# YamaneKoyo/mri-to-speech

Hardware: AMD Instinct MI355X
Metric: rtMRI frames/s end-to-end (256x256 frames -> 64-bin mel -> 11413 Hz wav) (higher is better)
Workload: dtype bf16x3; 1 GPU; e2e rtMRI->wav, 64 clips x 30 frames per GPU at 256x256 (configs[3] per-GPU share); clips_per_gpu=64, frames_per_clip=30, global_batch_clips=64, hw=256, parallelism=dp1, chunk=1920

## Files before the change

### mri-to-speech_amd/csrc/conv_gemm.hip

```cpp
#include "conv_igemm.hpp"

#include <cstring>
#include <map>
#include <mutex>

#include "prof.hpp"

namespace m2s {
namespace {

__device__ __attribute__((aligned(16))) uint4 g_zero_page[4];

template <int N>
__device__ __forceinline__ void wait_vm() {
  asm volatile("s_waitcnt vmcnt(%0)" ::"n"(N) : "memory");
}

__device__ __forceinline__ void dma16(const void* src, void* lds_wave_base) {
  __builtin_amdgcn_global_load_lds(src, lds_wave_base, 16, 0, 0);
}

__device__ __forceinline__ bf16x8 lrelu_frag(bf16x8 v, float slope) {
  uint4 u = __builtin_bit_cast(uint4, v);
  uint32_t w[4] = {u.x, u.y, u.z, u.w};
// ... 82 lines not shown
}

__device__ __forceinline__ void ld4f(const bf16_t* p, float* v) {
  const uint2 u = *reinterpret_cast<const uint2*>(p);
  v[0] = __uint_as_float(u.x << 16);
  v[1] = __uint_as_float(u.x & 0xffff0000u);
  v[2] = __uint_as_float(u.y << 16);
  v[3] = __uint_as_float(u.y & 0xffff0000u);
}

constexpr int ROW = 64;

__device__ __forceinline__ int swz_f(int x) { return (0x1320 >> (4 * x)) & 3; }
__device__ __forceinline__ int swz(int row, int chunk) { return row * ROW + ((chunk ^ swz_f((row >> 2) & 3)) << 4); }

template <int BM, int BN, int MT, int NT, int S, int KIND, int XF, int SP>
__global__ void __launch_bounds__(256, (BN >= 256 || (BM >= 256 && BN >= 128) ? 2 : 1)) conv_gemm_kernel(const ConvBatch ab, int n_tiles, int se_imgs,
                                                                                                      float* __restrict__ kpart) {
  const ConvArgs a = ab.a[KIND == KIND_CONV1D ? blockIdx.z : 0];
  constexpr int WN = BN / (NT * 16);
  constexpr int WM = 4 / WN;
  static_assert(WM * WN == 4 && WM * MT * 16 == BM, "bad tile");
  constexpr int R = SP == 1 ? 2 : 1;
  constexpr int A_PER_WAVE = BM / 64;
  constexpr int B_BLOCKS = BN / 16;
  constexpr int B_PER_WAVE = (B_BLOCKS + 3) / 4;
  constexpr int SLOT = (R * (BM + BN) + 16) * ROW;
  constexpr int PER_STAGE = R * (A_PER_WAVE + B_PER_WAVE);
  constexpr bool PRE = SP == 1 && XF == IN_SE_SCALE;
  constexpr bool SE = XF == IN_SE_SCALE;
  extern __shared__ __attribute__((aligned(16))) char smem[];
// ... 320 lines not shown
  }
  }

  if (nks > 1) {
    float* __restrict__ P = kpart + ((size_t)blockIdx.z * nks + ks) * a.M * a.cs_out;
#pragma unroll
    for (int mi = 0; mi < MT; ++mi) {
      const int m = m0 + wm * MT * 16 + mi * 16 + r16;
      if (m >= a.M) continue;
#pragma unroll
      for (int ni = 0; ni < NT; ++ni) {
        const int n4 = n0 + wn * NT * 16 + ni * 16 + 4 * g;
        if (n4 < a.cs_out)
          *reinterpret_cast<float4*>(P + (size_t)m * a.cs_out + n4) =
              make_float4(acc[ni][mi][0], acc[ni][mi][1], acc[ni][mi][2], acc[ni][mi][3]);
      }
    }
    return;
  }

  bf16_t* __restrict__ Y = static_cast<bf16_t*>(a.y);
  const bf16_t* __restrict__ Rs = static_cast<const bf16_t*>(a.res);
#pragma unroll
  for (int mi = 0; mi < MT; ++mi) {
    const int m = m0 + wm * MT * 16 + mi * 16 + r16;
    if (m >= a.M) continue;
    long orow;
    if constexpr (KIND == KIND_CONVT) {
      const int b = m / a.L_in, qq = m - (m / a.L_in) * a.L_in;
      orow = (long)b * a.L_out + (long)qq * a.ct_u + phase;
// ... 207 lines not shown
  }
  return static_cast<float*>(b.first);
}

const char* kname(int k) {
  switch (k) {
    case KIND_CONV2D: return "conv2d";
    case KIND_CONV1D: return "conv1d";
    case KIND_CONVT: return "convT";
    default: return "gemm";
  }
}

inline int se_images(int BM, int OH) { return BM % OH == 0 ? BM / OH : OH % BM == 0 ? 1 : (BM + OH - 1) / OH + 1; }

template <int BM, int BN, int MT, int NT, int KIND, int XF, int SP, int SF = 0>
void launch_tile(const ConvBatch& b, hipStream_t s, int phases, double flops, double bytes) {
  const ConvArgs& a = b.a[0];
  constexpr int S = SF ? SF : SP == 1 ? (BM == 128 && BN == 64 && XF != IN_SE_SCALE ? 3 : 2) : (BN >= 256 || BM + BN >= 384) ? 2 : (BM >= 256 ? 3 : 4);
  constexpr int R = SP == 1 ? 2 : 1;
  allow_lds(reinterpret_cast<const void*>(&conv_gemm_kernel<BM, BN, MT, NT, S, KIND, XF, SP>));
  const int m_tiles = ceil_div(a.M, BM), n_tiles = ceil_div(a.cs_out, BN);
  int se_imgs = 0;
  if (a.in_xform == IN_SE_SCALE) {
    M2S_CHECK(KIND == KIND_GEMM && a.OH > 0 && a.cs_in % 8 == 0, "SE scale needs the GEMM kind with OH = rows per image");
    se_imgs = se_images(BM, a.OH);
  }
  const size_t lds = (size_t)S * (R * (BM + BN) + 16) * ROW + (size_t)se_imgs * a.cs_in * sizeof(float);
  M2S_CHECK(lds <= 160 * 1024, "conv_gemm: LDS budget");
  int nst = 0;
  for (int i = 0; i < (KIND == KIND_CONV1D ? phases : 1); ++i) nst = std::max(nst, b.a[i].kp / 32);
  const int tiles = m_tiles * n_tiles * phases;
  const int slots = device_cus() * std::max(1, std::min(2, (int)(160 * 1024 / lds)));
  const char* fe = getenv("M2S_KSPLIT");
  const int force = fe ? atoi(fe) : 0;
  int nks = 1;
  if (force > 0)
    nks = std::min(force, std::max(1, nst));
  else if (2 * tiles <= slots && nst >= 8) {
    const char* mx = getenv("M2S_KSPLIT_MAX");
    const char* ms = getenv("M2S_KSPLIT_MINST");
    nks = std::max(1, std::min({slots / tiles, nst / (ms ? std::max(1, atoi(ms)) : 4), mx ? std::max(1, atoi(mx)) : 8}));
  }
  const size_t part_bytes = (size_t)phases * nks * a.M * a.cs_out * sizeof(float);
  if (nks > 1 && part_bytes > ((size_t)256 << 20)) nks = 1;
  float* kpart = nks > 1 ? ksplit_scratch(s, part_bytes) : nullptr;
  if (!kpart) nks = 1;
  dim3 grid(m_tiles * n_tiles, nks, phases);
  char name[96];
  static const bool detail = getenv("M2S_PROF_DETAIL") != nullptr;
  if (detail)
    snprintf(name, sizeof(name), "conv_gemm<%s,%dx%d%s> K%d N%d M%d", kname(KIND), BM, BN, SP == 1 ? ",x3" : SP == 2 ? ",e4m3" : "", a.kp, a.cs_out, a.M);
  else
    snprintf(name, sizeof(name), "conv_gemm_kernel<%d, %d, %d, %d, %d, %d, %d, %d>", BM, BN, MT, NT, S, KIND, XF, SP);
  {
    ProfScope ps(name, flops, bytes, s);
    hipLaunchKernelGGL((conv_gemm_kernel<BM, BN, MT, NT, S, KIND, XF, SP>), grid, dim3(256), lds, s, b, n_tiles, se_imgs, kpart);
  }
// ... 79 lines not shown
    const ConvArgs& c = as[i];
    M2S_CHECK(c.kind == a.kind && c.M == a.M && c.cs_in == a.cs_in && c.cs_out == a.cs_out && c.n_pad == a.n_pad &&
                  c.in_xform == a.in_xform && c.L_in == a.L_in && c.L_out == a.L_out,
              "conv_gemm batch: convs of one shape");
    M2S_CHECK(c.kp % 32 == 0 && c.kp >= c.ntaps * c.cs_in && c.ntaps <= 31, "conv_gemm batch: kp / taps");
    M2S_CHECK(c.x && c.w && c.bias && c.y && c.y != c.x && c.y != c.res, "conv_gemm batch: operand pointers");
    for (int j = 0; j < i; ++j) M2S_CHECK(as[j].y != c.y, "conv_gemm batch: two convs write one output");
    M2S_CHECK((double)(c.M / c.L_out) * c.L_in * c.cs_in * 2 < 2147483647.0, "conv_gemm batch: 32-bit offsets");
    b.a[i] = c;
  }
  if (a.M <= 0) return;
  launch_kind<KIND_CONV1D, 1>(a, s, n, flops, bytes, &b);
  M2S_HIP(hipGetLastError());
}

void launch_conv_gemm(const ConvArgs& a, bool split, hipStream_t s, double flops, double bytes) {
  M2S_CHECK(a.cs_in % 8 == 0 && a.cs_out % 4 == 0, "conv_gemm: channel strides");
  M2S_CHECK(a.cs_in >= 32 ? a.cs_in % 32 == 0 : 32 % a.cs_in == 0, "conv_gemm: channel stride vs the 32-wide K step");
  M2S_CHECK(a.ntaps <= 31, "conv_gemm: at most 31 taps");
  {
    const double in_elems = a.kind == KIND_CONV2D ? (double)(a.M / (a.OH * a.OW)) * a.IH * a.IW * a.cs_in
                            : a.kind == KIND_CONV1D ? (double)(a.M / a.L_out) * a.L_in * a.cs_in
                            : a.kind == KIND_CONVT  ? (double)a.M * a.cs_in
                                                    : (double)a.M * a.cs_in;
    M2S_CHECK(in_elems * (split ? 2 : 1) < 2147483647.0, "conv_gemm: input too large for 32-bit offsets (use a smaller chunk)");
  }
  M2S_CHECK(a.kp % 32 == 0 && a.kp >= a.ntaps * a.cs_in, "conv_gemm: kp");
  M2S_CHECK(a.kind != KIND_CONV2D || a.ks == 3, "conv_gemm: 2-D kernels are 3x3 (1x1 runs as GEMM)");
  if (a.M <= 0) return;
  M2S_CHECK(!(split && a.wscale), "conv_gemm: e4m3 operands take bf16 storage");
// ... 35 lines not shown
```

### mri-to-speech_amd/csrc/conv_igemm.hpp

```cpp
#pragma once

#include "m2s_common.hpp"

namespace m2s {

enum ConvKind { KIND_CONV2D = 0, KIND_CONV1D = 1, KIND_CONVT = 2, KIND_GEMM = 3 };
enum Act { ACT_NONE = 0, ACT_SILU = 1, ACT_LRELU = 2, ACT_SIGMOID = 3 };
enum InXform { IN_NONE = 0, IN_LRELU = 1, IN_SE_SCALE = 2 };

struct ConvArgs {
  const void* x;
  const void* w;
  const float* bias;
  const void* res;
  void* y;
  const void* in_scale;
  const float* wscale;
  int kind;
  int M;
  int cs_in, cs_out;
  int n_pad;
  int kp;
  int ntaps;
  int tpc;
// ... 5 lines not shown
  int accum;
  float accum_div;
  float res_unslope;
  int act_after_res;
  int kwave;
};

constexpr int CONV_BATCH = 3;
struct ConvBatch {
  ConvArgs a[CONV_BATCH];
};

template <typename T>
void launch_conv(const ConvArgs& a, hipStream_t s, double flops = 0.0, double bytes = 0.0);
void launch_conv_gemm(const ConvArgs& a, bool split, hipStream_t s, double flops, double bytes);
void launch_conv_gemm_batch(const ConvArgs* a, int n, hipStream_t s, double flops, double bytes);
bool conv_halo_supported(const ConvArgs& a);
void launch_conv_halo(const ConvArgs& a, hipStream_t s, double flops, double bytes);

inline int conv_tpc(int cs_in, int kc) { return cs_in < kc ? kc / cs_in : 1; }
inline int conv_kp(int ntaps, int cs_in, int kc) {
  int tpc = conv_tpc(cs_in, kc);
  return round_up(ntaps, tpc) * cs_in;
}

}
```

### mri-to-speech_amd/csrc/kernels.hpp

```cpp
#pragma once

#include "m2s_common.hpp"

namespace m2s {

enum AsyncCode : unsigned { M2S_ASYNC_LSTM = 1u, M2S_ASYNC_WS = 2u };
struct AsyncReport {
  unsigned spin_max = 1u << 20;
  unsigned* err = nullptr;
};
__device__ __forceinline__ void report_async(unsigned* err, unsigned code, int lane) {
  if (err && lane == 0) __hip_atomic_store(err, code, __ATOMIC_RELAXED, __HIP_MEMORY_SCOPE_SYSTEM);
}

template <typename T>
void launch_stem(const float* frames, int N, int H, int W, int OH, int OW, int pad_t, int pad_l,
                 const float* w9, const float* bias, int cout, int cs_out, T* y, hipStream_t s);

int dw_pixel_blocks(int OH, int OW);
template <typename T>
void launch_dwconv(const T* x, int N, int IH, int IW, int OH, int OW, int stride, int pad_t, int pad_l,
                   int C, int cs, const float* w9, const float* bias, T* y, float* sums, hipStream_t s);

template <typename T>
// ... 6 lines not shown
                    const void* w8 = nullptr, const float* wsc = nullptr, int kp8 = 0);
void launch_rows_e4m3(const void* x, long rows, int cs, void* y8, int ld8, hipStream_t s);

bool se_gemm_f8_supported(int P, int cs_in, int cs_out);
void launch_se_gemm_f8(const void* x8, int M, int P, int cs_in, const void* w8, int kp, int n_pad, const float* wscale,
                       const float* bias, const void* gate, const void* res, void* y, int cs_out, hipStream_t s,
                       double flops, double bytes, void* y8 = nullptr, int ld8 = 0);

bool se_gemm_sp_supported(int P, int cs_in, int cs_out);
void launch_se_gemm_sp(const void* x, int M, int P, int cs_in, const void* w, int n_pad, const float* bias,
                       const void* gate, const void* res, void* y, int cs_out, hipStream_t s, double flops, double bytes);

bool se_ws_supported(int P, int cs_in, int cs_out);
void launch_se_ws(const void* x, int M, int P, int cs_in, const void* w, int n_pad, const float* bias, const void* gate,
                  const void* res, void* y, int cs_out, hipStream_t s, double flops, double bytes, AsyncReport rep = {},
                  bool x_f32 = false);

bool se_ws_f8_supported(int P, int cs_in, int cs_out);
void launch_se_ws_f8(const void* x8, int M, int P, int cs_in, const void* w8, int kp, int n_pad, const float* wscale,
                     const float* bias, const void* gate, const void* res, void* y, int cs_out, hipStream_t s, double flops,
                     double bytes, void* y8 = nullptr, int ld8 = 0, AsyncReport rep = {});

bool ir_ws_supported(int H, int W, int cs_in, int kp, int cs_mid);
bool ir_ws_s2_supported(int H, int W, int cs_in, int kp, int cs_mid, int OH, int OW, int pad_t, int pad_l);
void launch_ir_ws(const void* x, int N, int H, int W, int cs_in, int kp, int cs_mid, const void* wpw, const float* bpw,
                  const float* wdw, const float* bdw, void* y, void* se_mean, double flops, double bytes,
                  hipStream_t s, AsyncReport rep = {}, int stride = 1, int OH = 0, int OW = 0, int pad_t = 0,
                  int pad_l = 0, double spill = 0.0, bool fm32 = false);
int ir_s2band_bands(int OH);
bool ir_s2band_supported(int IH, int IW, int OH, int OW, int cs_in, int kp, int cs_mid);
void launch_ir_s2band(const void* x, int N, int IH, int IW, int cs_in, int kp, const void* wpw, const float* bpw,
// ... 160 lines not shown
```

### mri-to-speech_amd/csrc/model.cpp

```cpp
#include "model.hpp"

#include <algorithm>
#include <cmath>
#include <cstdlib>
#include <cstring>
#include <initializer_list>
#include <type_traits>
#include <utility>

#include "pack.hpp"
#include "prof.hpp"

namespace m2s {

void Arena::upload(int device) {
  M2S_HIP(hipSetDevice(device));
  M2S_HIP(hipMalloc(&dev_, host_.size() + 256));
  M2S_HIP(hipMemcpy(dev_, host_.data(), host_.size(), hipMemcpyHostToDevice));
  std::vector<uint8_t>().swap(host_);
}

Arena::~Arena() {
  if (dev_) (void)hipFree(dev_);
}
// ... 2 lines not shown
  if (const char* e = std::getenv(name)) v = std::strcmp(e, "0") != 0;
}
static void env_int(const char* name, int& v) {
  if (const char* e = std::getenv(name)) v = std::atoi(e);
}

Acoustic::Acoustic(const StateDict& sd, int n_mels, int hidden, int dtype, int device)
    : dtype_(dtype), device_(device), n_mels_(n_mels), hidden_(hidden) {
  for (auto [name, v] : std::initializer_list<std::pair<const char*, bool*>>{
           {"M2S_IR_FUSED", &ir_fused_},   {"M2S_IR_WS", &ir_ws_},         {"M2S_IR_WS_S2", &ir_ws_s2_},
           {"M2S_IRWS_F32", &irws_f32_},   {"M2S_STEM_FUSED", &stem_fused_}, {"M2S_F8_EXPAND", &f8_expand_},
           {"M2S_F8_S2", &f8_s2_},         {"M2S_F8_ER", &f8_er_},         {"M2S_ER8_X8", &er8_x8_},
           {"M2S_F8_ER2", &f8_er2_},       {"M2S_SE_Y8", &se_y8_},         {"M2S_SE_FUSED", &se_fused_},
           {"M2S_ER_FUSED", &er_fused_},   {"M2S_SE_WS", &se_ws_},         {"M2S_LSTM_PERSISTENT", &lstm_persistent_},
           {"M2S_LSTM_MID", &lstm_mid_},   {"M2S_LSTM_X3", &lstm_x3_},     {"M2S_LSTM_X3G", &lstm_x3g_},
           {"M2S_SE_SP", &se_sp_},         {"M2S_ER_MRG", &er_mrg_},       {"M2S_IR_S2BAND", &ir_s2band_}})
    env_flag(name, *v);
  env_int("M2S_IRWS_MIN", irws_min_);
  env_int("M2S_SEWS_MIN", sews_min_cus_);
  pack_acoustic(sd, n_mels, hidden, dtype, arena_, p_);
  arena_.upload(device);
  for (auto& b : p_.blocks) {
    b.c1.resolve(arena_);
    if (b.type != 0) b.c2.resolve(arena_);
    if (b.type == 2) {
      b.se1.resolve(arena_);
      b.se2.resolve(arena_);
    }
  }
  p_.lstm_ih.resolve(arena_);
  M2S_HIP(hipHostMalloc(reinterpret_cast<void**>(&err_host_), sizeof(unsigned), hipHostMallocMapped | hipHostMallocCoherent));
// ... 161 lines not shown
  } else if (std::is_same<T, bf16_t>::value && er_fused_ && b.er_frag && b.stride == 2 &&
             ers2_fused_supported(nh, nw, b.c1.cs_in, b.mid, chan_stride(b.cout), b.c1.kp, b.c2.kp)) {
    uint8_t* y8 = er8_next && ((chan_stride(b.cout) == 32 && p_.blocks[k + 1].er8 && er8_fused_supported(nh, nw, 32, 128, 32)) ||
                               (chan_stride(b.cout) == 64 && p_.blocks[k + 1].er8w && er8w_fused_supported(nh, nw, 64, 224, b.cout)))
                      ? er8_next
                      : nullptr;
    launch_ers2_fused(reinterpret_cast<const bf16_t*>(cur), nc, oh, ow, nh, nw, qt, ql, b.c1.cs_in, b.mid,
                      chan_stride(b.cout), static_cast<const bf16_t*>(arena_.ptr(b.er_wexp)), b.c1.b,
                      static_cast<const bf16_t*>(arena_.ptr(b.er_wpwl)), b.c2.b, reinterpret_cast<bf16_t*>(nxt),
                      2.0 * px * b.mid * (9.0 * b.cin + b.cout),
                      2.0 * ((double)nc * oh * ow * b.c1.cs_in + px * chan_stride(b.cout)) + (y8 ? px * 32 : 0.0), s, y8);
    next8 = y8;
  } else {
    ConvArgs a = conv2d_args(p, b.c1, cur, M);
    a.act = ACT_SILU;
    run_conv<T>(a, b.c1, s);
    ConvArgs q = conv_args(b.c2);
    q.x = M;
    q.y = nxt;
    q.M = nc * nh * nw;
    q.OH = nh * nw;
    q.res = b.skip ? cur : nullptr;
    run_conv<T>(q, b.c2, s);
  }
}

template <typename T>
void Acoustic::effnet_ir_front(EffPass<T>& p, size_t k) {
  const Block& b = p_.blocks[k];
  const int nc = p.nc, oh = p.oh, ow = p.ow, nh = p.nh, nw = p.nw, qt = p.qt, ql = p.ql;
  T *const cur = p.cur, *const M = p.b.M, *const M2 = p.b.M2, *const se_mean = p.b.se_mean;
  float* const sums = p.b.sums;
  uint8_t *&cur8 = p.cur8, *const *const X8 = p.b.X8;
  hipStream_t s = p.s;
  const int cs = chan_stride(b.mid);
  constexpr bool SPL = std::is_same<T, sp_t>::value;
  const bool FUSABLE = (std::is_same<T, bf16_t>::value && (dtype_ == M2S_DT_BF16 || dtype_ == M2S_DT_FP8)) || SPL;
// ... 125 lines not shown
                        (next8 ? rows * b.cout : 0.0),
                    next8, ld8, ws_report());
  } else if (f8) {
    const double rows = (double)nc * nh * nw, co = chan_stride(b.cout);
    launch_se_gemm_f8(M2, nc * nh * nw, nh * nw, cs, arena_.ptr(b.f8_w), b.f8_kp, b.f8_npad,
                      static_cast<const float*>(arena_.ptr(b.f8_s)), static_cast<const float*>(arena_.ptr(b.f8_b)),
                      scale, b.skip ? cur : nullptr, nxt, chan_stride(b.cout), s, 2.0 * rows * b.mid * b.cout,
                      rows * cs + 2.0 * rows * co * (b.skip ? 2.0 : 1.0) + (double)b.f8_npad * b.f8_kp +
                          2.0 * nc * cs + (next8 ? rows * ld8 : 0.0),
                      next8, ld8);
  } else if (sews) {
    const double rows = (double)nc * nh * nw;
    launch_se_ws(M2, nc * nh * nw, nh * nw, cs, b.c2.w, b.c2.n_pad, b.c2.b, scale, b.skip ? cur : nullptr, nxt,
                 chan_stride(b.cout), s, 2.0 * rows * b.mid * b.cout,
                 4.0 * rows * b.mid + 4.0 * rows * b.cout * (b.skip ? 2.0 : 1.0) + 4.0 * b.cout * b.mid + 4.0 * nc * b.mid,
                 ws_report(), mid_f32);
  } else if (SPL && se_sp_ && se_gemm_sp_supported(nh * nw, cs, chan_stride(b.cout))) {
    const double rows = (double)nc * nh * nw, co = chan_stride(b.cout);
    launch_se_gemm_sp(M2, nc * nh * nw, nh * nw, cs, b.c2.w, b.c2.n_pad, b.c2.b, scale, b.skip ? cur : nullptr, nxt,
                      chan_stride(b.cout), s, 2.0 * rows * b.mid * b.cout,
                      4.0 * rows * cs + 4.0 * rows * co * (b.skip ? 2.0 : 1.0) + 4.0 * b.c2.n_pad * b.c2.kp +
                          4.0 * nc * cs);
  } else {
    ConvArgs q = conv_args(b.c2);
    q.x = M2;
    q.y = nxt;
    q.M = nc * nh * nw;
    q.OH = nh * nw;
    q.in_xform = IN_SE_SCALE;
    q.in_scale = scale;
    q.res = b.skip ? cur : nullptr;
// ... 979 lines not shown
```

### mri-to-speech_amd/csrc/model.hpp

```cpp
#pragma once

#include <map>
#include <string>
#include <vector>

#include "../../include/m2s.h"
#include "conv_igemm.hpp"
#include "kernels.hpp"

namespace m2s {

struct HostTensor {
  const float* data = nullptr;
  std::vector<int64_t> shape;
  size_t numel() const {
    size_t n = 1;
    for (auto d : shape) n *= (size_t)d;
    return n;
  }
};
using StateDict = std::map<std::string, HostTensor>;
StateDict make_state_dict(const m2s_tensor* t, int n);

class Arena {
// ... 196 lines not shown
  bool irws_f32_ = true;
  int sews_min_cus_ = 1;
  bool stem_fused_ = true;
  bool f8_er_ = true;
  bool se_y8_ = true;
  bool f8_er2_ = true;
  bool er8_x8_ = true;
  bool f8_expand_ = true;
  bool f8_s2_ = true;
  bool se_fused_ = true;
  bool er_fused_ = true;
  bool se_sp_ = false;
  bool se_ws_ = true;
  bool er_mrg_ = true;
  bool ir_s2band_ = true;
  bool lstm_persistent_ = true;
  bool lstm_mid_ = true;
  bool lstm_x3_ = true;
  bool lstm_x3g_ = true;

  size_t workspace_bytes(int B, int T, int H, int W) const;
  void forward(const float* frames, int B, int T, int H, int W, float* mel_norm, Workspace& ws, hipStream_t s);
  void effnet(const float* frames, int N, int H, int W, float* feats, int stop_after, float* probe, int* probe_dims,
              Workspace& ws, hipStream_t s);
  void bilstm(const float* feats, int B, int T, float* y, float* mel_norm, Workspace& ws, hipStream_t s);
  size_t ragged_workspace_bytes(const int* lengths, int B, int H, int W) const;
  void bilstm_ragged(const float* feats, const int* lengths, int B, long N, float* y, float* mel_norm, Workspace& ws,
                     hipStream_t s);
  void forward_ragged(const float* frames, const int* lengths, int B, long N, int H, int W, float* mel_norm,
                      Workspace& ws, hipStream_t s);
// ... 163 lines not shown
```

### mri-to-speech_amd/csrc/se_ws.hip

```cpp
#include <cstdlib>
#include <cstring>

#include "kernels.hpp"
#include "prof.hpp"

namespace m2s {
namespace {

typedef uint32_t u32x4 __attribute__((ext_vector_type(4)));

constexpr int ROWB = 128;

__device__ __attribute__((aligned(16))) uint4 g_se_ws_zero[4];


__device__ __forceinline__ void dma16(const void* src, uint32_t lds_wave_base) {
  unsigned keep;
  asm volatile("s_mov_b32 %0, m0\n\ts_mov_b32 m0, %2\n\ts_nop 0\n\tglobal_load_lds_dwordx4 %1, off\n\ts_mov_b32 m0, %0"
               : "=&s"(keep)
               : "v"(src), "s"(lds_wave_base)
               : "memory");
}
__device__ __forceinline__ uint32_t lds_u32(const void* p) { return (uint32_t)(uintptr_t)p; }

// ... 25 lines not shown
  unsigned spin_max;
  unsigned* err;
};

constexpr int E8M0_ONE = 0x7f7f7f7f;
typedef int i32x8 __attribute__((ext_vector_type(8)));
template <bool F8>
__device__ __forceinline__ int swz_k(int r) { return F8 ? (((r >> 1) & 1) | (r & 4)) : (r & 6); }
__device__ __forceinline__ int gate4_f8(int d, const float* s) {
  const f32x2_t lo = __builtin_amdgcn_cvt_pk_f32_fp8(d, false);
  const f32x2_t hi = __builtin_amdgcn_cvt_pk_f32_fp8(d, true);
  const int r = __builtin_amdgcn_cvt_pk_fp8_f32(lo[0] * s[0], lo[1] * s[1], 0, false);
  return __builtin_amdgcn_cvt_pk_fp8_f32(hi[0] * s[2], hi[1] * s[3], r, true);
}

template <int WM, int WN, int NT, int NL, int NS, int IF, bool F8, bool XF = false>
__global__ void __launch_bounds__(64 * (WM * WN + NL), 1) se_ws_kernel(const SeWsArgs a) {
  static_assert(!(F8 && XF), "fp32 activations: split engine");
  constexpr int NC = WM * WN;
  constexpr int BM = 64 * WM, BN = 16 * NT * WN, MT = 4;
  constexpr int BLK = (BN + BM) / 8;
  static_assert(BLK % NL == 0, "DMA blocks per loader");
  constexpr int PER = BLK / NL;
  static_assert((IF + 1) * PER <= 63 && IF >= 1 && IF <= NS - 1, "steps in flight per loader within vmcnt");
  constexpr int SLOT = (BN + BM) * ROWB;
  extern __shared__ __attribute__((aligned(16))) char smem[];

  const int tid = threadIdx.x, lane = tid & 63;
  const int wave = __builtin_amdgcn_readfirstlane(tid >> 6);
  const int nimg = BM / a.P > 0 ? BM / a.P : 1;
  const int grow = F8 ? a.cs_in * 2 : a.cs_in * 4;
  const int gimg = (grow + 1023) / 1024 * 1024;
  char* gbuf = smem + NS * SLOT;
  unsigned* flags = reinterpret_cast<unsigned*>(gbuf + 2 * nimg * gimg);
  const uint32_t full0 = lds_u32(flags), free0 = lds_u32(flags + NS), poison = lds_u32(flags + 2 * NS);
  const int nsteps = F8 ? a.kp / 128 : a.cs_in / 32;
  const int n_tiles = a.n_tiles_m;
  const int my_tiles = (int)blockIdx.x < n_tiles ? (n_tiles - 1 - (int)blockIdx.x) / (int)gridDim.x + 1 : 0;
  auto tile_rows = [&](int tile, int& m0, int& mend) {
    m0 = tile < a.full_tiles ? tile * BM : a.full_tiles * BM + (tile - a.full_tiles) * (BM / 2);
    mend = min(m0 + (tile < a.full_tiles ? BM : BM / 2), a.M);
  };

  if (tid <= 2 * NS) flags[tid] = 0u;
  __syncthreads();

  if (wave >= NC) {
    const int l = wave - NC;
    const char* zp = reinterpret_cast<const char*>(g_se_ws_zero);
    const int lrow = lane >> 3, pch = lane & 7;
    const int wrow_b = F8 ? a.kp : a.cs_in * 4, wlo = a.cs_in * 2, xrow_b = F8 ? a.cs_in : a.cs_in * 4;
    int s = 0;
    for (int it = 0; it < my_tiles; ++it) {
      const int tile = blockIdx.x + it * gridDim.x;
      int m0, mend;
      tile_rows(tile, m0, mend);
      const uint8_t* xt = a.x + (size_t)m0 * xrow_b;
      for (int st = 0; st < nsteps; ++st, ++s) {
        const int slot = s % NS, use = s / NS;
        if (use > 0 && !wait_flag(free0 + 4 * slot, (unsigned)(NC * use), a.spin_max)) {
          report_async(a.err, M2S_ASYNC_WS, lane);
          if (lane == 0) asm volatile("ds_write_b32 %0, %1\n\ts_waitcnt lgkmcnt(0)" ::"v"(poison), "v"(1u) : "memory");
        }
        if (st == 0 && l == 0) {
          const int img0 = m0 / a.P, nb = grow / 16;
          char* gdst = gbuf + (it & 1) * nimg * gimg;
          for (int im = 0; im < nimg; ++im)
            for (int o = 0; o < gimg / 16; o += 64) {
              const int e = o + lane;
// ... 39 lines not shown

  const int wm = wave / WN, wn = wave % WN;
  const int g = lane >> 4, r16 = lane & 15;
  const int sw = swz_k<F8>(r16);
  const uint32_t ch0 = (uint32_t)(((F8 ? 2 * g : g) ^ sw) << 4), ch1 = (uint32_t)(((F8 ? 2 * g + 1 : g + 4) ^ sw) << 4);
  const uint32_t sm0 = lds_u32(smem);
  const uint32_t a_lds0 = sm0 + (uint32_t)((wn * NT * 16 + r16) * ROWB);
  const uint32_t b_lds0 = sm0 + (uint32_t)((BN + wm * 64 + r16) * ROWB);
  const uint32_t bx0 = XF ? b_lds0 + (uint32_t)(((2 * g) ^ swz_k<true>(r16)) << 4) : 0u;
  const uint32_t bx1 = XF ? b_lds0 + (uint32_t)(((2 * g + 1) ^ swz_k<true>(r16)) << 4) : 0u;
  const uint32_t wa0 = XF ? a_lds0 + ch0 : 0u, wa1 = XF ? a_lds0 + ch1 : 0u;
  const uint32_t g_lds0 = lds_u32(gbuf) + (uint32_t)(g * (F8 ? 64 : 16));
  bool bad = false;
  int s = 0;
  for (int it = 0; it < my_tiles; ++it) {
    const int tile = blockIdx.x + it * gridDim.x;
    int m0, mend;
    tile_rows(tile, m0, mend);
    const bool active = m0 + wm * 64 < mend;
    const int wimg = (min(m0 + wm * 64, a.M - 1)) / a.P - m0 / a.P;
    const uint32_t gl = g_lds0 + (uint32_t)(((it & 1) * nimg + wimg) * gimg);
    f32x4 acc[NT][MT];
#pragma unroll
    for (int ni = 0; ni < NT; ++ni)
#pragma unroll
      for (int mi = 0; mi < MT; ++mi) acc[ni][mi] = f32x4{0.f, 0.f, 0.f, 0.f};

    for (int st = 0; st < nsteps; ++st, ++s) {
      const int slot = s % NS, use = s / NS;
      if (!wait_flag(full0 + 4 * slot, (unsigned)(NL * (use + 1)), a.spin_max)) {
        report_async(a.err, M2S_ASYNC_WS, lane);
// ... 210 lines not shown
        unpack_bf16x4(rv[mi & 1][ni][0], r);
        unpack_bf16x4(rv[mi & 1][ni][1], rl);
        float v[4] = {acc[ni][mi][0] + bb.x + (r[0] + rl[0]), acc[ni][mi][1] + bb.y + (r[1] + rl[1]),
                      acc[ni][mi][2] + bb.z + (r[2] + rl[2]), acc[ni][mi][3] + bb.w + (r[3] + rl[3])};
        if (bad) v[0] = v[1] = v[2] = v[3] = __builtin_nanf("");
        uint2 hi, lo;
        split4(v, hi, lo);
        bf16_t* yo = Y + (size_t)m * a.cs_out * 2 + n4;
        *reinterpret_cast<uint2*>(yo) = hi;
        *reinterpret_cast<uint2*>(yo + a.cs_out) = lo;
      }
    }
  }
}

template <int WM, int WN, int NT, int NL, int NS, int IF, bool F8 = false, bool XF = false>
void launch_cfg(SeWsArgs& a, hipStream_t s, double flops, double bytes) {
  static_assert(IF <= 3, "tail waits");
  constexpr int BM = 64 * WM, BN = 16 * NT * WN;
  const void* fn = reinterpret_cast<const void*>(&se_ws_kernel<WM, WN, NT, NL, NS, IF, F8, XF>);
  allow_lds(fn);
  const int nimg = BM / a.P > 0 ? BM / a.P : 1;
  const int gimg = ((F8 ? a.cs_in * 2 : a.cs_in * 4) + 1023) / 1024 * 1024;
  const size_t lds = (size_t)NS * (BN + BM) * ROWB + (size_t)2 * nimg * gimg + (2 * NS + 1) * sizeof(unsigned);
  M2S_CHECK(lds <= 160 * 1024, "se_ws: LDS budget");
  M2S_CHECK(BM % a.P == 0 || a.P % BM == 0, "se_ws: tile rows vs image size");
  M2S_CHECK(a.cs_out <= BN, "se_ws: one n tile covers the outputs");
  M2S_CHECK((F8 ? a.kp / 128 : a.cs_in / 32) >= NS, "se_ws: K steps per tile >= ring slots (gate rows are double-buffered per tile)");
  const int tiles = ceil_div(a.M, BM), G = std::min(tiles, device_cus());
  const int full = tiles / G * G, rem = tiles - full;
  const bool halve = rem > 0 && 2 * rem <= G && (BM / 2) % 64 == 0 && ((BM / 2) % a.P == 0 || a.P % (BM / 2) == 0) &&
                     getenv("M2S_SEWS_HALF") && atoi(getenv("M2S_SEWS_HALF")) == 1;
  a.full_tiles = halve ? full : tiles;
  a.n_tiles_m = halve ? full + 2 * rem : tiles;
  const dim3 grid(G);
  char name[72];
  if (XF)
    snprintf(name, sizeof(name), "se_ws_kernel<%d, %d, %d, %d, %d, %d, false, true>", WM, WN, NT, NL, NS, IF);
  else
    snprintf(name, sizeof(name), "se_ws_kernel<%d, %d, %d, %d, %d, %d, %s>", WM, WN, NT, NL, NS, IF,
             F8 ? "true" : "false");
  ProfScope ps(name, flops, bytes, s);
  hipLaunchKernelGGL((se_ws_kernel<WM, WN, NT, NL, NS, IF, F8, XF>), grid, dim3(64 * (WM * WN + NL)), lds, s, a);
  M2S_HIP(hipGetLastError());
}

}

bool se_ws_supported(int P, int cs_in, int cs_out) {
  return cs_in % 32 == 0 && cs_in / 32 >= 5 && ((P % 256 == 0 && cs_out <= 128) || (P == 64 && cs_out > 128 && cs_out <= 224));
}

void launch_se_ws(const void* x, int M, int P, int cs_in, const void* w, int n_pad, const float* bias, const void* gate,
                  const void* res, void* y, int cs_out, hipStream_t s, double flops, double bytes, AsyncReport rep,
                  bool x_f32) {
  M2S_CHECK(se_ws_supported(P, cs_in, cs_out) && M % P == 0 && cs_out % 4 == 0, "se_ws: unsupported shape");
  M2S_CHECK(x && w && bias && gate && y && y != res && y != x, "se_ws: operand pointers");
  M2S_CHECK((double)M * cs_in * 4 < 2147483647.0 * 2, "se_ws: input too large");
  if (M <= 0) return;
  SeWsArgs a;
  std::memset(&a, 0, sizeof(a));
  a.x = static_cast<const uint8_t*>(x);
  a.w = static_cast<const uint8_t*>(w);
  a.bias = bias;
  a.gate = static_cast<const uint8_t*>(gate);
  a.res = static_cast<const bf16_t*>(res);
  a.y = static_cast<bf16_t*>(y);
  a.M = M;
  a.P = P;
  a.cs_in = cs_in;
  a.cs_out = cs_out;
  a.spin_max = rep.spin_max;
  a.err = rep.err;
  static const int cfg = [] {
    const char* e = std::getenv("M2S_SE_WS_CFG");
    return e ? std::atoi(e) : 0;
  }();
  if (x_f32) {
    if (cs_out <= 128) {
      M2S_CHECK(n_pad >= 128, "se_ws: weight rows");
      return launch_cfg<4, 1, 8, 4, 3, 2, false, true>(a, s, flops, bytes);
    }
    M2S_CHECK(n_pad >= 224, "se_ws: weight rows");
    return launch_cfg<2, 2, 7, 4, 3, 2, false, true>(a, s, flops, bytes);
  }
  if (cs_out <= 128) {
    M2S_CHECK(n_pad >= 128, "se_ws: weight rows");
    switch (cfg) {
      case 1: return launch_cfg<4, 2, 4, 2, 3, 1>(a, s, flops, bytes);
      case 2: return launch_cfg<2, 2, 4, 4, 4, 2>(a, s, flops, bytes);
      case 3: return launch_cfg<2, 2, 4, 4, 4, 1>(a, s, flops, bytes);
      case 4: return launch_cfg<4, 2, 4, 4, 3, 2>(a, s, flops, bytes);
      default: return launch_cfg<4, 1, 8, 4, 3, 2>(a, s, flops, bytes);
    }
  } else {
    M2S_CHECK(n_pad >= 224, "se_ws: weight rows");
    switch (cfg) {
      case 1: return launch_cfg<2, 2, 7, 2, 3, 1>(a, s, flops, bytes);
      default: return launch_cfg<2, 2, 7, 4, 3, 2>(a, s, flops, bytes);
// ... 46 lines not shown
```

Baseline: 51080 rtMRI frames/s.

## Fuse stride-2 expand conv with projection GEMM and reverse se_ws tile walk

Adds an epilogue variant to the split 128x128 conv2d kernel that applies bias and SiLU to the expand-conv tile, stages it in LDS as hi/lo bf16, and runs the 1x1 projection GEMM in the same block. Stride-2 inverted-residual blocks then use one launch and skip the global round trip of the mid activation. Separately, the se_ws persistent kernel gains a REV template flag that walks tiles in reverse order, presumably to improve cache reuse with the preceding producer. Both are on by default. The fused path reloads projection weights from global per k-step and needs extra LDS reuse and registers, which may limit occupancy.

New measurement: 51830 rtMRI frames/s (median of 6 runs). 1.01x the previous value.

```diff
diff --git a/mri-to-speech_amd/csrc/conv_gemm.hip b/mri-to-speech_amd/csrc/conv_gemm.hip
--- a/mri-to-speech_amd/csrc/conv_gemm.hip
+++ b/mri-to-speech_amd/csrc/conv_gemm.hip
@@ -120,7 +120,7 @@
 __device__ __forceinline__ int swz_f(int x) { return (0x1320 >> (4 * x)) & 3; }
 __device__ __forceinline__ int swz(int row, int chunk) { return row * ROW + ((chunk ^ swz_f((row >> 2) & 3)) << 4); }
 
-template <int BM, int BN, int MT, int NT, int S, int KIND, int XF, int SP>
+template <int BM, int BN, int MT, int NT, int S, int KIND, int XF, int SP, int EP = 0>
 __global__ void __launch_bounds__(256, (BN >= 256 || (BM >= 256 && BN >= 128) ? 2 : 1)) conv_gemm_kernel(const ConvBatch ab, int n_tiles, int se_imgs,
                                                                                                       float* __restrict__ kpart) {
   const ConvArgs a = ab.a[KIND == KIND_CONV1D ? blockIdx.z : 0];
@@ -471,6 +471,87 @@
         if (n4 < a.cs_out)
           *reinterpret_cast<float4*>(P + (size_t)m * a.cs_out + n4) =
               make_float4(acc[ni][mi][0], acc[ni][mi][1], acc[ni][mi][2], acc[ni][mi][3]);
+      }
+    }
+    return;
+  }
+
+  if constexpr (EP == 1) {
+    static_assert(KIND == KIND_CONV2D && SP == 1 && XF == IN_NONE && BM == 128 && BN == 128 && MT == 4 && NT == 4,
+                  "the fused conv_pwl epilogue is built for the split 128 x 128 2-D tile");
+    static_assert((BN / 32) * 2 * BM * ROW <= S * SLOT, "the mid tile fits the ring");
+    constexpr int KS2 = BN / 32, NT2 = 2;
+    const bf16_t* __restrict__ W2 = static_cast<const bf16_t*>(ab.a[1].w);
+    const float* __restrict__ bias2 = ab.a[1].bias;
+    bf16_t* __restrict__ Y2 = static_cast<bf16_t*>(ab.a[1].y);
+    const int cs2 = ab.a[1].cs_out;
+    bf16x8 wh[2][NT2], wl[2][NT2];
+    auto load_w2 = [&](int kk) {
+#pragma unroll
+      for (int ni = 0; ni < NT2; ++ni) {
+        const bf16_t* p = W2 + (size_t)(wn * NT2 * 16 + ni * 16 + r16) * (2 * BN) + kk * 32 + g * 8;
+        wh[kk & 1][ni] = *reinterpret_cast<const bf16x8*>(p);
+        wl[kk & 1][ni] = *reinterpret_cast<const bf16x8*>(p + BN);
+      }
+    };
+    load_w2(0);
+    __syncthreads();
+#pragma unroll
+    for (int mi = 0; mi < MT; ++mi)
+#pragma unroll
+      for (int ni = 0; ni < NT; ++ni) {
+        const int row = wm * MT * 16 + mi * 16 + r16, n4 = wn * NT * 16 + ni * 16 + 4 * g;
+        const float4 bb = *reinterpret_cast<const float4*>(a.bias + n4);
+        float v[4] = {acc[ni][mi][0] + bb.x, acc[ni][mi][1] + bb.y, acc[ni][mi][2] + bb.z, acc[ni][mi][3] + bb.w};
+#pragma unroll
+        for (int j = 0; j < 4; ++j) v[j] = silu(v[j]);
+        asm volatile("" : "+v"(v[0]), "+v"(v[1]), "+v"(v[2]), "+v"(v[3]));
+        uint2 hi, lo;
+        split4(v, hi, lo);
+        char* d = smem + (n4 >> 5) * 2 * BM * ROW + swz(row, (n4 >> 3) & 3) + (n4 & 4) * 2;
+        *reinterpret_cast<uint2*>(d) = hi;
+        *reinterpret_cast<uint2*>(d + BM * ROW) = lo;
+      }
+    __syncthreads();
+    f32x4 acc2[NT2][MT];
+#pragma unroll
+    for (int ni = 0; ni < NT2; ++ni)
+#pragma unroll
+      for (int mi = 0; mi < MT; ++mi) acc2[ni][mi] = f32x4{0.f, 0.f, 0.f, 0.f};
+#pragma unroll
+    for (int kk = 0; kk < KS2; ++kk) {
+      const char* P = smem + kk * 2 * BM * ROW;
+      if (kk + 1 < KS2) load_w2(kk + 1);
+      bf16x8 bx[MT], bxl[MT];
+#pragma unroll
+      for (int mi = 0; mi < MT; ++mi) {
+        bx[mi] = *reinterpret_cast<const bf16x8*>(P + swz(wm * MT * 16 + mi * 16 + r16, g));
+        bxl[mi] = *reinterpret_cast<const bf16x8*>(P + BM * ROW + swz(wm * MT * 16 + mi * 16 + r16, g));
+      }
+#pragma unroll
+      for (int ni = 0; ni < NT2; ++ni)
+#pragma unroll
+        for (int mi = 0; mi < MT; ++mi) {
+          acc2[ni][mi] = __builtin_amdgcn_mfma_f32_16x16x32_bf16(wl[kk & 1][ni], bx[mi], acc2[ni][mi], 0, 0, 0);
+          acc2[ni][mi] = __builtin_amdgcn_mfma_f32_16x16x32_bf16(wh[kk & 1][ni], bxl[mi], acc2[ni][mi], 0, 0, 0);
+          acc2[ni][mi] = __builtin_amdgcn_mfma_f32_16x16x32_bf16(wh[kk & 1][ni], bx[mi], acc2[ni][mi], 0, 0, 0);
+        }
+    }
+#pragma unroll
+    for (int mi = 0; mi < MT; ++mi) {
+      const int m = m0 + wm * MT * 16 + mi * 16 + r16;
+      if (m >= a.M) continue;
+#pragma unroll
+      for (int ni = 0; ni < NT2; ++ni) {
+        const int n4 = wn * NT2 * 16 + ni * 16 + 4 * g;
+        if (n4 >= cs2) continue;
+        const float4 bb = *reinterpret_cast<const float4*>(bias2 + n4);
+        const float v[4] = {acc2[ni][mi][0] + bb.x, acc2[ni][mi][1] + bb.y, acc2[ni][mi][2] + bb.z, acc2[ni][mi][3] + bb.w};
+        uint2 hi, lo;
+        split4(v, hi, lo);
+        bf16_t* yo = Y2 + (size_t)m * cs2 * 2 + n4;
+        *reinterpret_cast<uint2*>(yo) = hi;
+        *reinterpret_cast<uint2*>(yo + cs2) = lo;
       }
     }
     return;
@@ -708,6 +789,21 @@
 
 inline int se_images(int BM, int OH) { return BM % OH == 0 ? BM / OH : OH % BM == 0 ? 1 : (BM + OH - 1) / OH + 1; }
 
+int plan_ksplit(int tiles, int nst, size_t lds) {
+  const int slots = device_cus() * std::max(1, std::min(2, (int)(160 * 1024 / lds)));
+  const char* fe = getenv("M2S_KSPLIT");
+  const int force = fe ? atoi(fe) : 0;
+  int nks = 1;
+  if (force > 0)
+    nks = std::min(force, std::max(1, nst));
+  else if (2 * tiles <= slots && nst >= 8) {
+    const char* mx = getenv("M2S_KSPLIT_MAX");
+    const char* ms = getenv("M2S_KSPLIT_MINST");
+    nks = std::max(1, std::min({slots / tiles, nst / (ms ? std::max(1, atoi(ms)) : 4), mx ? std::max(1, atoi(mx)) : 8}));
+  }
+  return nks;
+}
+
 template <int BM, int BN, int MT, int NT, int KIND, int XF, int SP, int SF = 0>
 void launch_tile(const ConvBatch& b, hipStream_t s, int phases, double flops, double bytes) {
   const ConvArgs& a = b.a[0];
@@ -724,18 +820,7 @@
   M2S_CHECK(lds <= 160 * 1024, "conv_gemm: LDS budget");
   int nst = 0;
   for (int i = 0; i < (KIND == KIND_CONV1D ? phases : 1); ++i) nst = std::max(nst, b.a[i].kp / 32);
-  const int tiles = m_tiles * n_tiles * phases;
-  const int slots = device_cus() * std::max(1, std::min(2, (int)(160 * 1024 / lds)));
-  const char* fe = getenv("M2S_KSPLIT");
-  const int force = fe ? atoi(fe) : 0;
-  int nks = 1;
-  if (force > 0)
-    nks = std::min(force, std::max(1, nst));
-  else if (2 * tiles <= slots && nst >= 8) {
-    const char* mx = getenv("M2S_KSPLIT_MAX");
-    const char* ms = getenv("M2S_KSPLIT_MINST");
-    nks = std::max(1, std::min({slots / tiles, nst / (ms ? std::max(1, atoi(ms)) : 4), mx ? std::max(1, atoi(mx)) : 8}));
-  }
+  int nks = plan_ksplit(m_tiles * n_tiles * phases, nst, lds);
   const size_t part_bytes = (size_t)phases * nks * a.M * a.cs_out * sizeof(float);
   if (nks > 1 && part_bytes > ((size_t)256 << 20)) nks = 1;
   float* kpart = nks > 1 ? ksplit_scratch(s, part_bytes) : nullptr;
@@ -845,6 +930,38 @@
   M2S_HIP(hipGetLastError());
 }
 
+namespace {
+constexpr int ER_BM = 128, ER_BN = 128, ER_S = 2;
+constexpr size_t ER_LDS = (size_t)ER_S * (2 * (ER_BM + ER_BN) + 16) * ROW;
+}
+
+bool conv_gemm_er_supported(const ConvArgs& e, const ConvArgs& q) {
+  const bool exp_ok = e.kind == KIND_CONV2D && e.ks == 3 && e.ntaps == 9 && e.cs_in >= 32 && e.cs_in % 32 == 0 &&
+                      e.kp % 32 == 0 && e.kp >= 9 * e.cs_in && e.cs_out == ER_BN && e.n_pad >= ER_BN && e.act == ACT_SILU &&
+                      !e.res && !e.accum && e.in_xform == IN_NONE && !e.wscale && e.M > 0 && e.OH > 0 && e.OW > 0 &&
+                      (double)(e.M / (e.OH * e.OW)) * e.IH * e.IW * e.cs_in * 2 < 2147483647.0;
+  const bool pwl_ok = q.kind == KIND_GEMM && q.cs_in == ER_BN && q.kp == ER_BN && q.cs_out % 4 == 0 && q.cs_out <= 64 &&
+                      q.n_pad >= 64 && q.act == ACT_NONE && !q.res && !q.accum && q.in_xform == IN_NONE && !q.wscale &&
+                      q.M == e.M;
+  return exp_ok && pwl_ok && plan_ksplit(ceil_div(e.M, ER_BM), e.kp / 32, ER_LDS) == 1;
+}
+
+void launch_conv_gemm_er(const ConvArgs& e, const ConvArgs& q, hipStream_t s, double flops, double bytes) {
+  M2S_CHECK(conv_gemm_er_supported(e, q), "conv_gemm_er: unsupported block");
+  M2S_CHECK(e.x && e.w && e.bias && q.w && q.bias && q.y && q.y != e.x, "conv_gemm_er: operand pointers");
+  ConvBatch b;
+  std::memset(&b, 0, sizeof(b));
+  b.a[0] = e;
+  b.a[1] = q;
+  auto* fn = &conv_gemm_kernel<ER_BM, ER_BN, 4, 4, ER_S, KIND_CONV2D, IN_NONE, 1, 1>;
+  allow_lds(reinterpret_cast<const void*>(fn));
+  char name[96];
+  snprintf(name, sizeof(name), "conv_gemm_kernel<%d, %d, 4, 4, %d, %d, %d, 1, 1>", ER_BM, ER_BN, ER_S, KIND_CONV2D, IN_NONE);
+  ProfScope ps(name, flops, bytes, s);
+  hipLaunchKernelGGL(fn, dim3(ceil_div(e.M, ER_BM), 1, 1), dim3(256), ER_LDS, s, b, 1, 0, static_cast<float*>(nullptr));
+  M2S_HIP(hipGetLastError());
+}
+
 void launch_conv_gemm(const ConvArgs& a, bool split, hipStream_t s, double flops, double bytes) {
   M2S_CHECK(a.cs_in % 8 == 0 && a.cs_out % 4 == 0, "conv_gemm: channel strides");
   M2S_CHECK(a.cs_in >= 32 ? a.cs_in % 32 == 0 : 32 % a.cs_in == 0, "conv_gemm: channel stride vs the 32-wide K step");
diff --git a/mri-to-speech_amd/csrc/conv_igemm.hpp b/mri-to-speech_amd/csrc/conv_igemm.hpp
--- a/mri-to-speech_amd/csrc/conv_igemm.hpp
+++ b/mri-to-speech_amd/csrc/conv_igemm.hpp
@@ -43,6 +43,8 @@
 template <typename T>
 void launch_conv(const ConvArgs& a, hipStream_t s, double flops = 0.0, double bytes = 0.0);
 void launch_conv_gemm(const ConvArgs& a, bool split, hipStream_t s, double flops, double bytes);
+bool conv_gemm_er_supported(const ConvArgs& e, const ConvArgs& q);
+void launch_conv_gemm_er(const ConvArgs& e, const ConvArgs& q, hipStream_t s, double flops, double bytes);
 void launch_conv_gemm_batch(const ConvArgs* a, int n, hipStream_t s, double flops, double bytes);
 bool conv_halo_supported(const ConvArgs& a);
 void launch_conv_halo(const ConvArgs& a, hipStream_t s, double flops, double bytes);
diff --git a/mri-to-speech_amd/csrc/kernels.hpp b/mri-to-speech_amd/csrc/kernels.hpp
--- a/mri-to-speech_amd/csrc/kernels.hpp
+++ b/mri-to-speech_amd/csrc/kernels.hpp
@@ -44,7 +44,7 @@
 bool se_ws_supported(int P, int cs_in, int cs_out);
 void launch_se_ws(const void* x, int M, int P, int cs_in, const void* w, int n_pad, const float* bias, const void* gate,
                   const void* res, void* y, int cs_out, hipStream_t s, double flops, double bytes, AsyncReport rep = {},
-                  bool x_f32 = false);
+                  bool x_f32 = false, bool rev = false);
 
 bool se_ws_f8_supported(int P, int cs_in, int cs_out);
 void launch_se_ws_f8(const void* x8, int M, int P, int cs_in, const void* w8, int kp, int n_pad, const float* wscale,
diff --git a/mri-to-speech_amd/csrc/model.cpp b/mri-to-speech_amd/csrc/model.cpp
--- a/mri-to-speech_amd/csrc/model.cpp
+++ b/mri-to-speech_amd/csrc/model.cpp
@@ -40,7 +40,8 @@
            {"M2S_F8_ER2", &f8_er2_},       {"M2S_SE_Y8", &se_y8_},         {"M2S_SE_FUSED", &se_fused_},
            {"M2S_ER_FUSED", &er_fused_},   {"M2S_SE_WS", &se_ws_},         {"M2S_LSTM_PERSISTENT", &lstm_persistent_},
            {"M2S_LSTM_MID", &lstm_mid_},   {"M2S_LSTM_X3", &lstm_x3_},     {"M2S_LSTM_X3G", &lstm_x3g_},
-           {"M2S_SE_SP", &se_sp_},         {"M2S_ER_MRG", &er_mrg_},       {"M2S_IR_S2BAND", &ir_s2band_}})
+           {"M2S_SE_SP", &se_sp_},         {"M2S_ER_MRG", &er_mrg_},       {"M2S_IR_S2BAND", &ir_s2band_},
+           {"M2S_ER_S2_FUSED", &er_s2_fused_}, {"M2S_SEWS_REV", &sews_rev_}})
     env_flag(name, *v);
   env_int("M2S_IRWS_MIN", irws_min_);
   env_int("M2S_SEWS_MIN", sews_min_cus_);
@@ -232,13 +233,18 @@
   } else {
     ConvArgs a = conv2d_args(p, b.c1, cur, M);
     a.act = ACT_SILU;
-    run_conv<T>(a, b.c1, s);
     ConvArgs q = conv_args(b.c2);
     q.x = M;
     q.y = nxt;
     q.M = nc * nh * nw;
     q.OH = nh * nw;
     q.res = b.skip ? cur : nullptr;
+    if (std::is_same<T, sp_t>::value && er_s2_fused_ && b.stride == 2 && conv_gemm_er_supported(a, q)) {
+      launch_conv_gemm_er(a, q, s, 2.0 * px * b.mid * (9.0 * b.cin + b.cout),
+                          4.0 * ((double)nc * oh * ow * b.cin + px * b.cout + (9.0 * b.cin + b.cout) * b.mid));
+      return;
+    }
+    run_conv<T>(a, b.c1, s);
     run_conv<T>(q, b.c2, s);
   }
 }
@@ -394,7 +400,7 @@
     launch_se_ws(M2, nc * nh * nw, nh * nw, cs, b.c2.w, b.c2.n_pad, b.c2.b, scale, b.skip ? cur : nullptr, nxt,
                  chan_stride(b.cout), s, 2.0 * rows * b.mid * b.cout,
                  4.0 * rows * b.mid + 4.0 * rows * b.cout * (b.skip ? 2.0 : 1.0) + 4.0 * b.cout * b.mid + 4.0 * nc * b.mid,
-                 ws_report(), mid_f32);
+                 ws_report(), mid_f32, sews_rev_);
   } else if (SPL && se_sp_ && se_gemm_sp_supported(nh * nw, cs, chan_stride(b.cout))) {
     const double rows = (double)nc * nh * nw, co = chan_stride(b.cout);
     launch_se_gemm_sp(M2, nc * nh * nw, nh * nw, cs, b.c2.w, b.c2.n_pad, b.c2.b, scale, b.skip ? cur : nullptr, nxt,
diff --git a/mri-to-speech_amd/csrc/model.hpp b/mri-to-speech_amd/csrc/model.hpp
--- a/mri-to-speech_amd/csrc/model.hpp
+++ b/mri-to-speech_amd/csrc/model.hpp
@@ -234,6 +234,8 @@
   bool se_ws_ = true;
   bool er_mrg_ = true;
   bool ir_s2band_ = true;
+  bool er_s2_fused_ = true;
+  bool sews_rev_ = true;
   bool lstm_persistent_ = true;
   bool lstm_mid_ = true;
   bool lstm_x3_ = true;
diff --git a/mri-to-speech_amd/csrc/se_ws.hip b/mri-to-speech_amd/csrc/se_ws.hip
--- a/mri-to-speech_amd/csrc/se_ws.hip
+++ b/mri-to-speech_amd/csrc/se_ws.hip
@@ -63,7 +63,7 @@
   return __builtin_amdgcn_cvt_pk_fp8_f32(hi[0] * s[2], hi[1] * s[3], r, true);
 }
 
-template <int WM, int WN, int NT, int NL, int NS, int IF, bool F8, bool XF = false>
+template <int WM, int WN, int NT, int NL, int NS, int IF, bool REV, bool F8, bool XF = false>
 __global__ void __launch_bounds__(64 * (WM * WN + NL), 1) se_ws_kernel(const SeWsArgs a) {
   static_assert(!(F8 && XF), "fp32 activations: split engine");
   constexpr int NC = WM * WN;
@@ -90,6 +90,10 @@
     m0 = tile < a.full_tiles ? tile * BM : a.full_tiles * BM + (tile - a.full_tiles) * (BM / 2);
     mend = min(m0 + (tile < a.full_tiles ? BM : BM / 2), a.M);
   };
+  auto walk = [&](int it) -> int {
+    const int t = blockIdx.x + it * gridDim.x;
+    return REV ? n_tiles - 1 - t : t;
+  };
 
   if (tid <= 2 * NS) flags[tid] = 0u;
   __syncthreads();
@@ -101,7 +105,7 @@
     const int wrow_b = F8 ? a.kp : a.cs_in * 4, wlo = a.cs_in * 2, xrow_b = F8 ? a.cs_in : a.cs_in * 4;
     int s = 0;
     for (int it = 0; it < my_tiles; ++it) {
-      const int tile = blockIdx.x + it * gridDim.x;
+      const int tile = walk(it);
       int m0, mend;
       tile_rows(tile, m0, mend);
       const uint8_t* xt = a.x + (size_t)m0 * xrow_b;
@@ -171,7 +175,7 @@
   bool bad = false;
   int s = 0;
   for (int it = 0; it < my_tiles; ++it) {
-    const int tile = blockIdx.x + it * gridDim.x;
+    const int tile = walk(it);
     int m0, mend;
     tile_rows(tile, m0, mend);
     const bool active = m0 + wm * 64 < mend;
@@ -412,11 +416,11 @@
   }
 }
 
-template <int WM, int WN, int NT, int NL, int NS, int IF, bool F8 = false, bool XF = false>
+template <int WM, int WN, int NT, int NL, int NS, int IF, bool F8 = false, bool XF = false, bool REV = false>
 void launch_cfg(SeWsArgs& a, hipStream_t s, double flops, double bytes) {
   static_assert(IF <= 3, "tail waits");
   constexpr int BM = 64 * WM, BN = 16 * NT * WN;
-  const void* fn = reinterpret_cast<const void*>(&se_ws_kernel<WM, WN, NT, NL, NS, IF, F8, XF>);
+  const void* fn = reinterpret_cast<const void*>(&se_ws_kernel<WM, WN, NT, NL, NS, IF, REV, F8, XF>);
   allow_lds(fn);
   const int nimg = BM / a.P > 0 ? BM / a.P : 1;
   const int gimg = ((F8 ? a.cs_in * 2 : a.cs_in * 4) + 1023) / 1024 * 1024;
@@ -433,13 +437,15 @@
   a.n_tiles_m = halve ? full + 2 * rem : tiles;
   const dim3 grid(G);
   char name[72];
-  if (XF)
+  if (REV)
+    snprintf(name, sizeof(name), "se_ws_kernel<%d, %d, %d, %d, %d, %d, true, false%s>", WM, WN, NT, NL, NS, IF, XF ? ", true" : "");
+  else if (XF)
     snprintf(name, sizeof(name), "se_ws_kernel<%d, %d, %d, %d, %d, %d, false, true>", WM, WN, NT, NL, NS, IF);
   else
     snprintf(name, sizeof(name), "se_ws_kernel<%d, %d, %d, %d, %d, %d, %s>", WM, WN, NT, NL, NS, IF,
              F8 ? "true" : "false");
   ProfScope ps(name, flops, bytes, s);
-  hipLaunchKernelGGL((se_ws_kernel<WM, WN, NT, NL, NS, IF, F8, XF>), grid, dim3(64 * (WM * WN + NL)), lds, s, a);
+  hipLaunchKernelGGL((se_ws_kernel<WM, WN, NT, NL, NS, IF, REV, F8, XF>), grid, dim3(64 * (WM * WN + NL)), lds, s, a);
   M2S_HIP(hipGetLastError());
 }
 
@@ -451,7 +457,7 @@
 
 void launch_se_ws(const void* x, int M, int P, int cs_in, const void* w, int n_pad, const float* bias, const void* gate,
                   const void* res, void* y, int cs_out, hipStream_t s, double flops, double bytes, AsyncReport rep,
-                  bool x_f32) {
+                  bool x_f32, bool rev) {
   M2S_CHECK(se_ws_supported(P, cs_in, cs_out) && M % P == 0 && cs_out % 4 == 0, "se_ws: unsupported shape");
   M2S_CHECK(x && w && bias && gate && y && y != res && y != x, "se_ws: operand pointers");
   M2S_CHECK((double)M * cs_in * 4 < 2147483647.0 * 2, "se_ws: input too large");
@@ -477,10 +483,17 @@
   if (x_f32) {
     if (cs_out <= 128) {
       M2S_CHECK(n_pad >= 128, "se_ws: weight rows");
+      if (rev) return launch_cfg<4, 1, 8, 4, 3, 2, false, true, true>(a, s, flops, bytes);
       return launch_cfg<4, 1, 8, 4, 3, 2, false, true>(a, s, flops, bytes);
     }
     M2S_CHECK(n_pad >= 224, "se_ws: weight rows");
+    if (rev) return launch_cfg<2, 2, 7, 4, 3, 2, false, true, true>(a, s, flops, bytes);
     return launch_cfg<2, 2, 7, 4, 3, 2, false, true>(a, s, flops, bytes);
+  }
+  if (rev && cfg == 0) {
+    M2S_CHECK(n_pad >= (cs_out <= 128 ? 128 : 224), "se_ws: weight rows");
+    if (cs_out <= 128) return launch_cfg<4, 1, 8, 4, 3, 2, false, false, true>(a, s, flops, bytes);
+    return launch_cfg<2, 2, 7, 4, 3, 2, false, false, true>(a, s, flops, bytes);
   }
   if (cs_out <= 128) {
     M2S_CHECK(n_pad >= 128, "se_ws: weight rows");
```
